# KTC-Security-Circle/3d-matching

Measured on AMD Instinct MI355X. Metric: ICP iterations/sec + RANSAC hypotheses/sec, 100k↔100k pts, 1/2/4/8 GPU, higher is better.
Workload: dtype fp16-split MFMA NN screen + fp32 scan, exact fp64 NN decision, fp64 terms/solve; 1 GPU; cfg1: 100000<->100000 synthetic pair per GPU, 50 point-to-plane ICP iterations, brute-force NN (r=0.12), 1 GPU; ns=100000, nt_per_gpu=100000, parallelism=single, comm=none, comm_ranks=1

## Files before the change

### 3d-matching_amd/csrc/api.cpp

```cpp
#include <cfloat>
#include <chrono>
#include <hip/hip_runtime.h>
#include <string.h>

#include <algorithm>
#include <cmath>
#include <string>
#include <memory>
#include <mutex>
#include <unordered_map>
#include <vector>

#include "linalg.h"
#include "m3d_internal.h"
#include "ddmath.h"

using namespace m3d;

int m3d_fail(m3d_ctx* ctx, int code, const std::string& msg) {
  if (ctx) ctx->err = msg;
  return code;
}

KTimer::KTimer(m3d_ctx* c, int kid, hipStream_t s) : ctx(c), id(kid), st(s) {
// ... 1261 lines not shown
      if (e != hipSuccess) grc = m3d_fail(ctx, M3D_ERR_HIP, std::string("grid fp64 points: ") + hipGetErrorString(e));
    }
    if (!grc && params->nn_method == M3D_NN_BRUTE && tg->mf16 == nullptr) {
      hipError_t e = build_mfma_tiles(tgt, const_cast<Grid*>(tg), &ctx->tmp, nullptr);
      if (e != hipSuccess) grc = m3d_fail(ctx, M3D_ERR_HIP, std::string("mfma tiles: ") + hipGetErrorString(e));
    }
    if (!grc) {
      cand_cap = heavy_cap(params, coarse_max_occ);
      const size_t n1 = (size_t)std::max<int64_t>(src->n, 1);
      Carve cv;
      cv.add(&s->state, 1);
      if (params->nn_method == M3D_NN_BRUTE) nn_plan_shape(src->n, &s->nn_qblocks, &s->nn_budget);
      if (s->nn_qblocks > 0) {
        cv.add(&s->nn_cnt, (size_t)s->nn_qblocks);
        cv.add(&s->nn_seen, (size_t)s->nn_qblocks);
        cv.add(&s->nn_table, (size_t)s->nn_budget);
      }
      cv.add(&s->keys, n1);
      cv.add(&s->near2, n1);
      cv.add(&s->dprev, n1);
      cv.add(&s->ld64, n1);
      cv.add(&s->lidx, n1);
      cv.add(&s->corr, n1);
      cv.add(&s->partials, (size_t)(terms_blocks(src->n) * kTermSlots + kTermSlots));
      if (cand_cap > 0) {
        cv.add(&s->hlist, n1);
        cv.add(&s->hcnt, kDeferWords);
        s->hcap = (int32_t)n1;
      }
      cv.add(&s->pcd64, 3 * n1);
      size_t tot = 0;
      hipError_t e = run_arena ? ctx->run.reserve(cv.bytes()) : cv.alloc(&s->block, &tot, nullptr);
      if (e != hipSuccess) grc = m3d_fail(ctx, M3D_ERR_OOM, "device allocation failed (ICP loop arrays)");
      if (!grc && run_arena) cv.place(ctx->run.base);
    }
    if (!grc && s->hcnt != nullptr &&
        hipMemsetAsync(s->hcnt, 0, kDeferWords * sizeof(uint32_t), nullptr) != hipSuccess)
      grc = m3d_fail(ctx, M3D_ERR_HIP, "loop arrays: deferral counter");
    if (!grc && s->nn_cnt != nullptr &&
        hipMemsetAsync(s->nn_cnt, 0, (size_t)s->nn_qblocks * sizeof(uint32_t), nullptr) != hipSuccess)
      grc = m3d_fail(ctx, M3D_ERR_HIP, "loop arrays: NN plan counters");
    if (!grc) {
      hipError_t e = hipStreamSynchronize(nullptr);
      if (e != hipSuccess) grc = m3d_fail(ctx, M3D_ERR_HIP, std::string("loop setup: ") + hipGetErrorString(e));
    }
    if (grc) {
// ... 1217 lines not shown
  const int32_t forced = 2;
  HIPX(s->ctx, hipMemcpyAsync(s->nn_table, table.data(), sizeof(uint32_t) * table.size(), hipMemcpyHostToDevice, S(stream)));
  HIPX(s->ctx, hipMemcpyAsync(&s->state->plan_ok, &forced, sizeof(forced), hipMemcpyHostToDevice, S(stream)));
  HIPX(s->ctx, hipStreamSynchronize(S(stream)));
  return M3D_OK;
}

int m3d_debug_icp_nn_plan_read(m3d_icp* s, uint32_t* counts, uint32_t* table, int32_t* shape3, void* stream) {
  if (!s || !shape3) return M3D_ERR_INVALID;
  shape3[0] = s->nn_qblocks;
  shape3[1] = s->nn_budget;
  shape3[2] = 0;
  if (s->nn_qblocks <= 0) return M3D_OK;
  Touch tch{s->ctx, S(stream)};
  if (counts)
    HIPX(s->ctx, hipMemcpyAsync(counts, s->nn_seen, sizeof(uint32_t) * (size_t)s->nn_qblocks, hipMemcpyDeviceToHost, S(stream)));
  if (table)
    HIPX(s->ctx, hipMemcpyAsync(table, s->nn_table, sizeof(uint32_t) * (size_t)s->nn_budget, hipMemcpyDeviceToHost, S(stream)));
  HIPX(s->ctx, hipMemcpyAsync(&shape3[2], &s->state->plan_ok, sizeof(int32_t), hipMemcpyDeviceToHost, S(stream)));
  HIPX(s->ctx, hipStreamSynchronize(S(stream)));
  return M3D_OK;
}

}
```

### 3d-matching_amd/csrc/icp.hip

```cpp
#include <float.h>

#include <algorithm>
#include <string>
#include <type_traits>
#include <vector>
#include <stdlib.h>

#include "lds_dma.h"
#include "linalg.h"
#include "m3d_internal.h"
#include "nnkey.h"

namespace m3d {

constexpr int kTermsBlock = 512;
constexpr double kU = 5.9604644775390625e-08;
constexpr double kU64 = 1.1102230246251565e-16;


struct FrameParams {
  double cs[3], ct[3];
  double pinf, qinf;
  double s16;
  int shared;
// ... 199 lines not shown
      for (int y = 0; y < 3; ++y) acc[6 + 3 * x + y] += pc[x] * qc[y];
    }
  }
}

struct TermsArgs {
  double* pcd64;
  const float4* src32;
  int64_t ns;
  const double* tgt64;
  const double* nrm64;
  const double* rec64;
  int64_t nt_shard, off;
  const int64_t* keys;
  uint32_t* near2;
  GridDev g;
  const int32_t* claim;
  const int64_t* dmin;
  int64_t* dprev;
  int32_t* corr;
  int est;
  double c[3];
  int64_t* reset_keys;
};

#if M3D_TAIL_CLOCK
__device__ unsigned long long g_tail_clock[3 * 4096 + 24];
#endif
#if M3D_TERMS_CLOCK
__device__ unsigned long long g_terms_clock[4096 * 8];
#define M3D_TPH(k)                               \
  do {                                           \
    __builtin_amdgcn_s_waitcnt(0);               \
    tph_[k] = __builtin_amdgcn_s_memrealtime();  \
  } while (0)
#else
#define M3D_TPH(k) \
  do {             \
  } while (0)
#endif
template <bool kWT, int kEst>
__device__ __forceinline__ void terms_block(const TermsArgs& a, const IcpState* __restrict__ s,
                                            double* __restrict__ partials) {
  __shared__ double red[kTermSlots][kTermsBlock / kWave];
#if M3D_TERMS_CLOCK
  unsigned long long tph_[8];
// ... 58 lines not shown
#endif
      qx[u] = qy[u] = qz[u] = 0.0f;
      if (amb[u]) xform32(s->Rt32, a.src32[ii[u]], qx[u], qy[u], qz[u]);
      bj[u] = -1;
      bd[u] = 0.0;
    }
    resolve_wave(amb[0], a.g, a.tgt64, a.off, qx[0], qy[0], qz[0], X[0], vs[0], s->r2, bj[0], bd[0]);
#pragma unroll
    for (int u = 0; u < kP; ++u) {
      if (amb[u]) {
        gj[u] = bj[u];
        d2[u] = bd[u];
      } else if (valid[u] && key_real(k1[u])) {
        const int64_t c = (int64_t)(uint32_t)k1[u];
        if (c >= a.off && c < a.off + a.nt_shard) {
          gj[u] = c;
          fixed[u] = false;
        }
      }
    }
  }
  M3D_TPH(2);
  double tq[kP][3], tn[kP][3];
#pragma unroll
  for (int u = 0; u < kP; ++u) {
    const bool own = valid[u] && gj[u] >= a.off && gj[u] < a.off + a.nt_shard;
    const int64_t l = own ? gj[u] - a.off : 0;
    if (a.nt_shard == 0) {
      for (int k = 0; k < 3; ++k) tq[u][k] = tn[u][k] = 0.0;
    } else if (a.rec64 != nullptr) {
      const double4 r0 = reinterpret_cast<const double4*>(a.rec64)[2 * l];
      const double4 r1 = reinterpret_cast<const double4*>(a.rec64)[2 * l + 1];
      tq[u][0] = r0.x;
      tq[u][1] = r0.y;
      tq[u][2] = r0.z;
      tn[u][0] = r0.w;
      tn[u][1] = r1.x;
      tn[u][2] = r1.y;
    } else {
#pragma unroll
      for (int k = 0; k < 3; ++k) {
        tq[u][k] = a.tgt64[3 * l + k];
        tn[u][k] = kEst == M3D_EST_POINT_TO_PLANE ? a.nrm64[3 * l + k] : 0.0;
      }
    }
  }
  M3D_TPH(3);
#pragma unroll
  for (int u = 0; u < kP; ++u) {
    if (!valid[u]) continue;
    if (!fixed[u]) {
      const double d = d2_64(vs[u], tq[u]);
      if (d < s->r2) {
        d2[u] = d;
      } else {
        gj[u] = -1;
      }
    }
    const int64_t i = ii[u];
    if (a.corr != nullptr) a.corr[i] = (int32_t)gj[u];
    if (gj[u] < a.off || gj[u] >= a.off + a.nt_shard) continue;
    terms_add<kEst>(acc, vs[u], tq[u], tn[u], d2[u], a.c);
  }
  M3D_TPH(4);
  const int lane = threadIdx.x & (kWave - 1), wave = threadIdx.x / kWave;
  {
    double v[32];
#pragma unroll
    for (int k = 0; k < 32; ++k) v[k] = k < 30 ? acc[k] : 0.0;
    const double w = wave_transpose_sum32(v, lane);
    if ((lane & 1) == 0) red[lane >> 1][wave] = w;
  }
  M3D_TPH(5);
  __syncthreads();
  M3D_TPH(6);
  if (threadIdx.x < kTermSlots) {
    double v = 0.0;
    if (threadIdx.x < 30)
      for (int w = 0; w < kTermsBlock / kWave; ++w) v += red[threadIdx.x][w];
    double* dst = partials + (int64_t)blockIdx.x * kTermSlots + threadIdx.x;
    if (kWT)
      __hip_atomic_store(reinterpret_cast<unsigned long long*>(dst), __double_as_longlong(v),
                         __ATOMIC_RELAXED, __HIP_MEMORY_SCOPE_AGENT);
// ... 665 lines not shown
  copy_points_kernel<<<(unsigned)((n + 255) / 256), 256, 0, st>>>(s->state, s->pcd64, s->src->slot, n, dst);
  return hipGetLastError();
}

hipError_t launch_val_states(const m3d_icp* s, const double* T_dev, const int32_t* list, int64_t n,
                             IcpState* states, hipStream_t st) {
  if (n == 0) return hipSuccess;
  val_states_kernel<<<(unsigned)((n + 63) / 64), 64, 0, st>>>(states, T_dev, list, n,
                                                              s->max_dist * s->max_dist, frame_of(s));
  return hipGetLastError();
}

hipError_t launch_icp_keyinit(const m3d_icp* s, int64_t off, hipStream_t st, int64_t q0, int64_t q1) {
  const int64_t ns = q1 < 0 ? s->src->n : q1;
  if (ns <= q0) return hipSuccess;
  keyinit_kernel<<<(unsigned)((ns - q0 + 255) / 256), 256, 0, st>>>(
      s->src->xyz32, ns, s->tgt->xyz32, s->tgt->n, off, s->state, s->corr, s->dprev, s->keys,
      s->near2, q0);
  return hipGetLastError();
}


__global__ __launch_bounds__(256) void pack_rec_kernel(const double* __restrict__ xyz,
                                                       const double* __restrict__ nrm, int64_t n,
                                                       double* __restrict__ rec) {
  const int64_t i = (int64_t)blockIdx.x * 256 + threadIdx.x;
  if (i >= n) return;
  double r[8];
  for (int k = 0; k < 3; ++k) {
    r[k] = xyz[3 * i + k];
    r[3 + k] = nrm != nullptr ? nrm[3 * i + k] : 0.0;
  }
  r[6] = r[7] = 0.0;
  for (int k = 0; k < 8; ++k) rec[8 * i + k] = r[k];
}

hipError_t ensure_target_rec(const m3d_cloud* c, hipStream_t st) {
  if (c->rec64 != nullptr || c->n == 0) return hipSuccess;
  double* rec = nullptr;
  hipError_t e = block_alloc(reinterpret_cast<void**>(&rec), sizeof(double) * 8 * c->n, st);
  if (e != hipSuccess) return e;
  pack_rec_kernel<<<(unsigned)((c->n + 255) / 256), 256, 0, st>>>(c->xyz64, c->nrm64, c->n, rec);
  e = hipGetLastError();
  if (e != hipSuccess) {
    block_release(rec);
    return e;
  }
  c->rec64 = rec;
  return hipSuccess;
}

__global__ __launch_bounds__(256) void pack_pts64_kernel(const float4* __restrict__ pts,
                                                         const double* __restrict__ xyz, int64_t n,
                                                         double4* __restrict__ out) {
  const int64_t k = (int64_t)blockIdx.x * 256 + threadIdx.x;
  if (k >= n) return;
  const int32_t j = __float_as_int(pts[k].w);
  out[k] = make_double4(xyz[3 * (int64_t)j], xyz[3 * (int64_t)j + 1], xyz[3 * (int64_t)j + 2],
                        __longlong_as_double((long long)j));
}

hipError_t build_grid_pts64(const m3d_cloud* c, Grid* g, hipStream_t st) {
  if (g->pts64 != nullptr || g->n_pts == 0) return hipSuccess;
  double4* p = nullptr;
  hipError_t e = block_alloc(reinterpret_cast<void**>(&p), sizeof(double4) * g->n_pts, st);
// ... 10 lines not shown
}

static TermsArgs terms_args(const m3d_icp* s, int64_t off, const int32_t* claim,
                            const int64_t* dmin, bool reset_keys) {
  TermsArgs a;
  a.pcd64 = s->pcd64;
  a.src32 = s->src->xyz32;
  a.ns = s->src->n;
  a.tgt64 = s->tgt->xyz64;
  a.nrm64 = s->tgt->nrm64;
  a.rec64 = s->tgt->rec64;
  a.nt_shard = s->tgt->n;
  a.off = off;
  a.keys = s->keys;
  a.near2 = s->near2;
  a.g = s->tgrid->dev;
  a.claim = claim;
  a.dmin = dmin;
  a.dprev = claim != nullptr ? s->dprev : nullptr;
  a.corr = s->corr;
  a.est = s->params.estimation;
  for (int k = 0; k < 3; ++k) a.c[k] = s->src->center[k];
  a.reset_keys = reset_keys ? s->keys : nullptr;
  return a;
}

hipError_t launch_icp_terms_mode(const m3d_icp* s, int64_t off, const int32_t* claim,
                                 const int64_t* dmin, hipStream_t st) {
  const int64_t ns = s->src->n;
  if (ns == 0) return hipMemsetAsync(s->partials, 0, sizeof(double) * kTermSlots, st);
  const TermsArgs ta = terms_args(s, off, claim, dmin, false);
  const unsigned nb = (unsigned)s->nblocks;
  with_est(ta.est, [&](auto e) {
    terms_kernel<decltype(e)::value><<<nb, kTermsBlock, 0, st>>>(ta, s->state, s->partials);
  });
  return hipGetLastError();
}

static void launch_reduce_groups(const m3d_icp* s, double* sums, int do_solve, hipStream_t st) {
  const SolveParams sp = do_solve ? solve_params(s) : SolveParams{};
  with_est(do_solve ? s->params.estimation : M3D_EST_POINT_TO_PLANE, [&](auto e) {
    reduce_groups_kernel<decltype(e)::value><<<kReduceGroups, kTermSlots, 0, st>>>(
        s->partials, s->nblocks, sums, s->state, sp, do_solve);
  });
}

// ... 135 lines not shown
```

### 3d-matching_amd/csrc/m3d_internal.h

```cpp
#pragma once

#include <hip/hip_runtime.h>
#include <stdint.h>

#include <algorithm>
#include <string>
#include <utility>
#include <functional>
#include <memory>
#include <mutex>
#include <vector>

#include "../../include/m3d.h"
#include "nn_plan.h"

#define M3D_CONST __attribute__((address_space(4)))

namespace m3d {

constexpr int kWave = 64;

struct alignas(64) HypF32 {
  float r[9];
  float t[3];
// ... 243 lines not shown
  const m3d_cloud* user_src = nullptr;
  const m3d_cloud* tgt = nullptr;
  m3d_icp_params params{};
  double max_dist = 0.0;
  void* block = nullptr;
  m3d::IcpState* state = nullptr;
  int64_t* keys = nullptr;
  uint32_t* near2 = nullptr;
  int64_t* dprev = nullptr;
  int64_t* ld64 = nullptr;
  int32_t* lidx = nullptr;
  int32_t* hlist = nullptr;
  uint32_t* hcnt = nullptr;
  int32_t hcap = 0;
  int32_t cand_cap = 0;
  int32_t scan_xchunk = 0;
  bool keys_clean = false;
  uint32_t* nn_cnt = nullptr;
  uint32_t* nn_seen = nullptr;
  uint32_t* nn_table = nullptr;
  int32_t nn_qblocks = 0;
  int32_t nn_budget = 0;
  int32_t* corr = nullptr;
  double* pcd64 = nullptr;
  double* partials = nullptr;
  double* sums = nullptr;
  int64_t nblocks = 0;
  const m3d::Grid* sgrid = nullptr;
  const m3d::Grid* tgrid = nullptr;
  int64_t ns_total = 0;
  bool xready_tgt = false;
  bool xready_src = false;
  int64_t* xdk = nullptr;
  int32_t* xcl = nullptr;
  double* xsums = nullptr;
  hipStream_t cap_stream = nullptr;
  hipGraphExec_t graph[2] = {nullptr, nullptr};
  int32_t graph_n[2] = {-1, -1};
  bool graph_kc_out[2] = {false, false};
  int32_t seen_n[2] = {-1, -1};
  bool graph_off = false;
};

int m3d_fail(m3d_ctx* ctx, int code, const std::string& msg);

struct KTimer {
// ... 197 lines not shown
```

### 3d-matching_amd/csrc/nn_brute.hip

```cpp
#include <algorithm>

#include "lds_dma.h"
#include "m3d_internal.h"
#include "nnkey.h"

#ifndef M3D_NN_BRUTE_PLAN_TU
#define M3D_NN_BRUTE_PLAN_TU 0
#endif
#ifndef M3D_NN_CLOCK
#define M3D_NN_CLOCK 0
#endif
#define M3D_NN_TU_MAIN (!M3D_NN_BRUTE_PLAN_TU)
#define M3D_NN_TU_PLAN_KERNEL (M3D_NN_BRUTE_PLAN_TU ? !M3D_NN_CLOCK : M3D_NN_CLOCK)
#if M3D_NN_TU_MAIN || M3D_NN_TU_PLAN_KERNEL

namespace m3d {

typedef _Float16 half8 __attribute__((ext_vector_type(8)));
typedef float floatx16 __attribute__((ext_vector_type(16)));

constexpr int kMG = 2;
constexpr int kMTile = 256;
constexpr int kTH = 4;
constexpr int kMTilePad = 1024;
// ... 112 lines not shown
    block_release(g->mf32);
    block_release(g->mfbox);
    g->mf16 = nullptr;
    g->mf32 = nullptr;
    g->mfbox = nullptr;
    return e;
  }
  g->mf_npad = n_pad;
  pack16_sorted_kernel<<<(unsigned)((n_pad + 255) / 256), 256, 0, st>>>(
      g->pts, perm, c->xyz32, n, n_pad, (float)c->s16, g->mf16, g->mf32);
  tile_box_kernel<<<(unsigned)(n_pad / kMTile), kMTile, 0, st>>>(g->mf32, g->mfbox);
  return hipGetLastError();
}

#endif

struct SeedArgs {
  const int32_t* prev;
  const float4* tgt;
  int64_t nt;
  int on;
};

__device__ __forceinline__ int64_t start_key(const SeedArgs& sa, const IcpState* __restrict__ s,
                                             int64_t i, float4 p, float qx, float qy, float qz,
                                             int64_t off, const int64_t* __restrict__ keys) {
  return sa.on ? seed_key(s, i, p, qx, qy, qz, sa.tgt, sa.nt, off, sa.prev, nullptr) : keys[i];
}

struct NnSlice {
  unsigned x, y, S;
};
struct NnPlan {
  const uint32_t* table;
  uint32_t* cnt;
  int nq, S;
};

__device__ __forceinline__ bool publish_k1(const SeedArgs& sa, unsigned y, uint64_t k1, bool changed) {
  return changed || (sa.on && y == 0 && key_real(k1));
}

__device__ void nn_slice_scan(const float4* __restrict__ src32, int64_t ns, const float4* __restrict__ tgt32,
                              int64_t jb, int64_t je, int64_t off, const IcpState* __restrict__ s,
                              int64_t* __restrict__ keys, uint32_t* __restrict__ near2,
                              const SeedArgs& sa, int64_t q0, unsigned bsx, unsigned bsy) {
  const float* Rt = s->Rt32;
  const float r2_hi = s->r2_hi;
  for (int qs = threadIdx.x; qs < kMQueries; qs += kMBlock) {
    const int64_t slot = q0 + (int64_t)bsx * kMQueries + qs;
    if (slot >= ns) return;
    const int64_t i = slot;
    float qx, qy, qz;
    const float4 p = src32[i];
    xform32(Rt, p, qx, qy, qz);
    const int64_t key = start_key(sa, s, i, p, qx, qy, qz, off, keys);
    uint64_t k1 = key == kKeyNone ? make_key(r2_hi, 0xFFFFFFFFu) : (uint64_t)key;
    float k1d = key_real_d2(k1), n2 = kInf;
    const uint64_t k10 = k1;
    for (int64_t j = jb; j < je; ++j) {
      const float4 t = tgt32[j];
      if (__float_as_int(t.w) < 0) continue;
      const float d2 = d2f(qx, qy, qz, t.x, t.y, t.z);
      if (d2 <= r2_hi) near_push(k1, k1d, n2, make_key(d2, (uint32_t)(off + __float_as_int(t.w))), d2);
    }
    const bool pk = publish_k1(sa, bsy, k1, k1 != k10);
    if (pk || n2 < kInf) near_publish((unsigned long long*)&keys[i], &near2[i], k1, n2, pk);
  }
}

__device__ __forceinline__ void nn_push_rows(const float4 (&t)[16], int64_t off, float qx, float qy, float qz,
                                             float r2_hi, uint64_t& k1, float& k1d, float& n2) {
#pragma unroll
  for (int reg = 0; reg < 16; ++reg) {
    const float d2 = d2f(qx, qy, qz, t[reg].x, t[reg].y, t[reg].z);
    const uint64_t kc = make_key(d2, (uint32_t)(off + __float_as_int(t[reg].w)));
    if (d2 <= r2_hi) near_push(k1, k1d, n2, kc, d2);
  }
}
// ... 21 lines not shown
  x |= __builtin_amdgcn_mov_dpp(x, 0x128, 0xF, 0xF, false);
  return (uint32_t)(__builtin_amdgcn_readlane(x, 0) | __builtin_amdgcn_readlane(x, 16) |
                    __builtin_amdgcn_readlane(x, 32) | __builtin_amdgcn_readlane(x, 48));
}

template <bool kMax>
__device__ __forceinline__ float wave_minmax(float v) {
  const auto mm = [](float a, float b) { return kMax ? fmaxf(a, b) : fminf(a, b); };
  v = mm(v, __int_as_float(__builtin_amdgcn_mov_dpp(__float_as_int(v), 0xB1, 0xF, 0xF, false)));
  v = mm(v, __int_as_float(__builtin_amdgcn_mov_dpp(__float_as_int(v), 0x4E, 0xF, 0xF, false)));
  v = mm(v, __int_as_float(xor4_dpp(__float_as_int(v))));
  v = mm(v, __int_as_float(__builtin_amdgcn_mov_dpp(__float_as_int(v), 0x128, 0xF, 0xF, false)));
  const int x = __float_as_int(v);
  return mm(mm(__int_as_float(__builtin_amdgcn_readlane(x, 0)), __int_as_float(__builtin_amdgcn_readlane(x, 16))),
            mm(__int_as_float(__builtin_amdgcn_readlane(x, 32)), __int_as_float(__builtin_amdgcn_readlane(x, 48))));
}

#ifndef M3D_NN_CULL
#define M3D_NN_CULL 1
#endif
#ifndef M3D_NN_REACH
#define M3D_NN_REACH 1
#endif
#ifndef M3D_NN_DEFER_BATCH
#define M3D_NN_DEFER_BATCH 1
#endif
#ifndef M3D_NN_DEFER_FILTER
#define M3D_NN_DEFER_FILTER 1
#endif
#if M3D_NN_CLOCK
constexpr int kClkBlocks = 16384, kClkWords = 8;
__device__ unsigned long long g_nn_clock[kClkWords * kClkBlocks];
#endif
struct QBox {
  float lo[3], hi[3], X;
};
__device__ __forceinline__ bool box_out_of_reach(const QBox& q, const float4& tlo, const float4& thi) {
  const float gx = fmaxf(0.0f, fmaxf(q.lo[0] - thi.x, tlo.x - q.hi[0]));
  const float gy = fmaxf(0.0f, fmaxf(q.lo[1] - thi.y, tlo.y - q.hi[1]));
  const float gz = fmaxf(0.0f, fmaxf(q.lo[2] - thi.z, tlo.z - q.hi[2]));
  return d2f(gx, gy, gz, 0.0f, 0.0f, 0.0f) > q.X;
}
__device__ __forceinline__ bool point_out_of_reach(float qx, float qy, float qz, float X, const float (&lo)[3],
                                                   const float (&hi)[3]) {
  const float gx = fmaxf(0.0f, fmaxf(qx - hi[0], lo[0] - qx));
  const float gy = fmaxf(0.0f, fmaxf(qy - hi[1], lo[1] - qy));
// ... 6 lines not shown
constexpr uint64_t kGMask = (kSub == 64) ? ~0ull : ((1ull << kSub) - 1ull);
constexpr int kDefer = 16;
static_assert(kMBlock == 2 * kMTile, "one 16-B operand half per thread per half tile");
static_assert(kSub * kMG <= 64, "hit mask holds every (group, sub-tile)");
static_assert(kSub == 32, "one 32-bit hit record per group and tile");
static_assert(kMBlock / 64 == 8, "eight wave boxes, lanes ^1 ^2 ^4");

struct QState {
  float qx, qy, qz, qq;
  int64_t qi;
  uint64_t k1;
  float k1d, n2;
  half8 bq;
};

__device__ __forceinline__ uint64_t group_mask(uint32_t bits) {
  uint64_t m = 0;
#pragma unroll
  for (int g = 0; g < kMG; ++g)
    if ((bits >> g) & 1u) m |= kGMask << (g * kSub);
  return m;
}

__device__ __forceinline__ float load_query(QState& q, QBox& lq, int64_t slot, int h,
                                            const float4* __restrict__ src32, int64_t ns,
                                            const IcpState* __restrict__ s, const SeedArgs& sa, int64_t off,
                                            const int64_t* __restrict__ keys) {
  const float* Rt = s->Rt32;
  const float r2_hi = s->r2_hi, S = s->mfma_scale;
  const int64_t i = slot < ns ? slot : -1;
  q.qi = i;
  q.n2 = kInf;
  float X = -1.0f;
  if (i >= 0) {
    const float4 p = src32[i];
    xform32(Rt, p, q.qx, q.qy, q.qz);
    const int64_t key = start_key(sa, s, i, p, q.qx, q.qy, q.qz, off, keys);
    q.k1 = key == kKeyNone ? make_key(r2_hi, 0xFFFFFFFFu) : (uint64_t)key;
    X = search_bound(key_d2(q.k1), s->band_e, r2_hi);
    lq.lo[0] = fminf(lq.lo[0], q.qx);
    lq.lo[1] = fminf(lq.lo[1], q.qy);
    lq.lo[2] = fminf(lq.lo[2], q.qz);
    lq.hi[0] = fmaxf(lq.hi[0], q.qx);
    lq.hi[1] = fmaxf(lq.hi[1], q.qy);
    lq.hi[2] = fmaxf(lq.hi[2], q.qz);
    lq.X = fmaxf(lq.X, X);
  } else {
    q.qx = q.qy = q.qz = 0.0f;
    q.k1 = (uint64_t)kKeyNone;
  }
  q.k1d = key_real_d2(q.k1);
  q.qq = fmaf(q.qz, q.qz, fmaf(q.qy, q.qy, q.qx * q.qx));
  _Float16 ah, al, bh, bl, ch, cl;
  split16(-2.0f * S * q.qx, ah, al);
  split16(-2.0f * S * q.qy, bh, bl);
  split16(-2.0f * S * q.qz, ch, cl);
  const _Float16 one = (_Float16)1.0f, zero = (_Float16)0.0f;
  q.bq = h == 0 ? half8{ah, al, ah, bh, bl, bh, ch, cl} : half8{ch, one, one, zero, zero, zero, zero, zero};
  return X;
}
// ... 195 lines not shown
  uint32_t m = 0;
#pragma unroll
  for (int reg = 15; reg >= 0; --reg) m = __builtin_amdgcn_alignbit(m, __float_as_uint(v[reg]), 31);
  return m;
}
__device__ __forceinline__ void nn_push_hits(uint32_t m, const float4* rows, int64_t off, int h, float qx,
                                             float qy, float qz, float r2_hi, uint64_t& k1, float& k1d,
                                             float& n2) {
  while (m != 0) {
    const int reg = __builtin_ctz(m);
    m &= m - 1;
    const float4 t = rows[(reg & 3) + 8 * (reg >> 2) + 4 * h];
    push_within(k1, k1d, n2, d2f(qx, qy, qz, t.x, t.y, t.z), r2_hi, (uint32_t)(off + __float_as_int(t.w)));
  }
}

template <bool kPlan>
__device__ __forceinline__ void nn_mfma_body(const float4* __restrict__ src32, int64_t ns,
                                             const uint4* __restrict__ tgt16, const float4* __restrict__ tgt32,
                                             const float4* __restrict__ tbox, int64_t nt_pad, int64_t off,
                                             const IcpState* __restrict__ s, int64_t* __restrict__ keys,
                                             uint32_t* __restrict__ near2, const SeedArgs& sa, int64_t q0,
                                             const NnPlan& pl) {
  if (s->done) return;
#if M3D_NN_CLOCK
  const unsigned long long clk0 = __builtin_amdgcn_s_memrealtime();
#endif
  NnSlice bs{0u, 0u, 0u};
  if (kPlan && pl.table != nullptr) {
    if (s->plan_ok) {
      const uint32_t e = pl.table[blockIdx.x];
      if (e == kPlanEmpty) return;
      bs = NnSlice{plan_x(e), plan_y(e), plan_S(e)};
    } else {
      const unsigned y = blockIdx.x / (unsigned)pl.nq;
      if (y >= (unsigned)pl.S) return;
      bs = NnSlice{blockIdx.x - y * (unsigned)pl.nq, y, (unsigned)pl.S};
    }
  }
  if (!s->mfma_ok) {
    const int64_t tstep = (int64_t)(kPlan ? bs.S : gridDim.y) * kTT;
    for (int64_t t0 = (int64_t)(kPlan ? bs.y : blockIdx.y) * kTT; t0 < nt_pad; t0 += tstep)
      nn_slice_scan(src32, ns, tgt32, t0, min(nt_pad, t0 + kTT), off, s, keys, near2, sa, q0,
                    kPlan ? bs.x : blockIdx.x, kPlan ? bs.y : blockIdx.y);
    return;
  }
  __shared__ uint4 t16[2][2][kTT];
  __shared__ uint64_t dlist[kMBlock / 64][kDefer];
  __shared__ uint32_t dtile[kMBlock / 64][kDefer];
  __shared__ float4 qbox[kMBlock / 64][2];
  __shared__ uint64_t rslot[2][kMBlock / 64];
#if M3D_NN_CLOCK
  __shared__ uint32_t clk_slow, clk_ticket;
  __shared__ unsigned long long clk_exit;
  if (threadIdx.x == 0) {
    clk_slow = 0;
    clk_ticket = 0;
    clk_exit = 0;
  }
  uint32_t clk_halves = 0;
#endif
  uint32_t kept = 0;
  __shared__ uint32_t slice_xy;
  if (kPlan && threadIdx.x == 0) slice_xy = bs.x | (bs.y << 16);
  const int lane = threadIdx.x & 63, wave = threadIdx.x >> 6;
  const int c = lane & 31, h = lane >> 5;
  const float r2_hi = s->r2_hi, eps = s->screen_eps_m, S = s->mfma_scale, be = s->band_e;
  const float S2 = S * S;

  QState q[kMG];
  uint32_t act = 0;
  uint32_t force = 0;
  uint32_t chg = 0;
  QBox lq{{kInf, kInf, kInf}, {-kInf, -kInf, -kInf}, -1.0f};
#pragma unroll
  for (int g = 0; g < kMG; ++g) {
    const int64_t slot = q0 + (kPlan ? (int64_t)bs.x : (int64_t)blockIdx.x) * kMQueries + (wave * kMG + g) * 32 + c;
    const float X = load_query(q[g], lq, slot, h, src32, ns, s, sa, off, keys);
    if (q[g].qi >= 0) act |= 1u << g;
    if (__any(refresh_threshold(q[g], h, X, eps, S2))) force |= 1u << g;
  }
  const floatx16 zacc = {0.0f, 0.0f, 0.0f, 0.0f, 0.0f, 0.0f, 0.0f, 0.0f,
                         0.0f, 0.0f, 0.0f, 0.0f, 0.0f, 0.0f, 0.0f, 0.0f};
  uint32_t dfr = 0;
#pragma unroll
  for (int g = 0; g < kMG; ++g)
    if (!((force >> g) & 1u) && __all(q[g].qi < 0 || key_real(q[g].k1))) dfr |= 1u << g;
  int dn = 0;
  uint64_t dmask = group_mask(dfr);
  dmask = ((uint64_t)(uint32_t)__builtin_amdgcn_readfirstlane((int)(dmask >> 32)) << 32) |
          (uint32_t)__builtin_amdgcn_readfirstlane((int)(uint32_t)dmask);

  const QBox bx = reduce_boxes(lq, qbox, lane, wave);
  const int ntile = (int)(nt_pad / kTT);
  const ReachArgs ra{q, act, be, r2_hi, rslot, wave};
  TileCursor cur{tbox, qbox[wave], bx, lane, ntile, (int)(kPlan ? bs.S : gridDim.y), (int)(kPlan ? bs.y : blockIdx.y), 0, 0};
  cur.cull_round(ra);
  int t0, t1;
  uint32_t h0, h1;
  cur.next(t0, h0, ra);
  if (t0 < ntile) stage_tile(t16[0], tgt16, nt_pad, t0, false);
// ... 256 lines not shown
  return hipMemcpyFromSymbol(out, HIP_SYMBOL(m3d::g_nn_clock), sizeof(unsigned long long) * (size_t)n) == hipSuccess ? 0 : -1;
}
namespace m3d {
#endif
static bool icp_nn_uses_mfma(const m3d_icp* s) {
  return s->tgrid != nullptr && s->tgrid->mf16 != nullptr;
}

bool icp_nn_range_ok(const m3d_icp* s) {
  if (s->params.nn_method == M3D_NN_GRID) return s->sgrid != nullptr && s->sgrid->mpts != nullptr;
  return icp_nn_uses_mfma(s);
}

hipError_t launch_icp_nn(const m3d_icp* s, int64_t off, bool self_seed, hipStream_t st, int64_t q0,
                         int64_t q1) {
  const int64_t ns = q1 < 0 ? s->src->n : q1;
  if (ns <= q0 || s->tgt->n == 0) return hipSuccess;
  const Grid* tg = s->tgrid;
  const int64_t tt = (int64_t)kTH * kMTile;
  if (!icp_nn_uses_mfma(s) || tg->mf_npad % tt != 0) return hipErrorInvalidValue;
  const int64_t slots = nn_resident_slots();
  const int64_t bx = (ns - q0 + kMQueries - 1) / kMQueries;
  const int64_t gy = nn_grid_y(bx, tg->mf_npad / tt, slots, M3D_NN_CULL != 0);
  const SeedArgs sa{s->corr, s->tgt->xyz32, s->tgt->n, self_seed ? 1 : 0};
  const bool planned = nn_plan_on() && s->nn_qblocks > 0 && q0 == 0 && ns == s->src->n && bx == s->nn_qblocks &&
                       bx * gy <= s->nn_budget;
  if (planned)
    return launch_nn_plan_kernel((unsigned)s->nn_budget, st, s->src->xyz32, ns, tg->mf16, tg->mf32, tg->mfbox,
                                 tg->mf_npad, off, s->state, s->keys, s->near2, sa, q0,
                                 NnPlan{s->nn_table, s->nn_cnt, (int)bx, (int)gy});
  nn_mfma_kernel<<<dim3((unsigned)bx, (unsigned)gy), kMBlock, 0, st>>>(
        s->src->xyz32, ns, tg->mf16, tg->mf32, tg->mfbox, tg->mf_npad, off, s->state, s->keys, s->near2, sa, q0);
  return hipGetLastError();
}

int64_t nn_resident_slots() {
  static const int64_t slots = [] {
    int dev = 0, per = 0;
    hipDeviceProp_t p;
    if (hipGetDevice(&dev) != hipSuccess || hipGetDeviceProperties(&p, dev) != hipSuccess) return (int64_t)0;
    if (hipOccupancyMaxActiveBlocksPerMultiprocessor(&per, nn_mfma_kernel, kMBlock, 0) != hipSuccess)
      return (int64_t)0;
    const int pp = nn_plan_kernel_blocks_per_cu();
    per = per > 0 ? per : 1;
    if (pp > 0 && pp < per) per = pp;
    return (int64_t)p.multiProcessorCount * per;
  }();
// ... 35 lines not shown
```

### 3d-matching_amd/csrc/nnkey.h

```cpp
#pragma once

#include <hip/hip_runtime.h>
#include <stdint.h>

#include "m3d_internal.h"

namespace m3d {

__device__ __forceinline__ float d2f(float qx, float qy, float qz, float tx, float ty, float tz) {
  const float dx = qx - tx, dy = qy - ty, dz = qz - tz;
  return fmaf(dz, dz, fmaf(dy, dy, dx * dx));
}

__device__ __forceinline__ void xform32(const float* Rt, float4 p, float& x, float& y, float& z) {
  x = fmaf(Rt[0], p.x, fmaf(Rt[1], p.y, fmaf(Rt[2], p.z, Rt[9])));
  y = fmaf(Rt[3], p.x, fmaf(Rt[4], p.y, fmaf(Rt[5], p.z, Rt[10])));
  z = fmaf(Rt[6], p.x, fmaf(Rt[7], p.y, fmaf(Rt[8], p.z, Rt[11])));
}

__device__ __forceinline__ void q64_of(const double* __restrict__ T, const double* __restrict__ p,
                                       double q[3]) {
  q[0] = ((T[0] * p[0] + T[1] * p[1]) + T[2] * p[2]) + T[3];
  q[1] = ((T[4] * p[0] + T[5] * p[1]) + T[6] * p[2]) + T[7];
  q[2] = ((T[8] * p[0] + T[9] * p[1]) + T[10] * p[2]) + T[11];
// ... 352 lines not shown
                                              const float4* __restrict__ tgt32, int64_t nt_shard,
                                              int64_t off, const int64_t* __restrict__ dprev) {
  if (j < 0) return kKeyNone;
  if (j >= off && j < off + nt_shard) {
    const float4 t = tgt32[j - off];
    const float d2 = d2f(qx, qy, qz, t.x, t.y, t.z);
    return d2 <= s->r2_hi ? (int64_t)make_key(d2, (uint32_t)j) : kKeyNone;
  }
  if (!s->bound_ok || dprev == nullptr) return kKeyNone;
  const int64_t dp = dprev[i];
  if (dp == kKeyNone) return kKeyNone;
  return bound_key(s, __double2float_ru(__longlong_as_double(dp)), p, qx, qy, qz);
}

__device__ __forceinline__ int64_t seed_key(const IcpState* __restrict__ s, int64_t i, float4 p,
                                            float qx, float qy, float qz,
                                            const float4* __restrict__ tgt32, int64_t nt_shard,
                                            int64_t off, const int32_t* __restrict__ prev,
                                            const int64_t* __restrict__ dprev) {
  if (prev == nullptr) return kKeyNone;
  return seed_key_j(s, (int64_t)prev[i], i, p, qx, qy, qz, tgt32, nt_shard, off, dprev);
}

}
```

### 3d-matching_amd/m3d/_lib.py

```python

from __future__ import annotations

import ctypes as C
import os
from pathlib import Path

LIB_PATH = Path(__file__).resolve().parent / "libm3d.so"

M3D_OK = 0
M3D_ERR_INVALID = -1
M3D_ERR_HIP = -2
M3D_ERR_OOM = -3
M3D_ERR_NODEVICE = -4
M3D_ERR_COMM = -5

HYP_OK, HYP_DEGENERATE, HYP_NONFINITE = 0, 1, 2
SCORE_SQUARED, SCORE_NORM = 0, 1
EST_POINT_TO_POINT, EST_POINT_TO_PLANE = 0, 1
KERNEL_NN, KERNEL_SCORE, KERNEL_KABSCH, KERNEL_TERMS, KERNEL_LOOP, KERNEL_COMM = 0, 1, 2, 3, 4, 5
ICP_NO_SPLIT = 2
NN_BRUTE, NN_GRID = 0, 1
EVAL_INFORMATION = 1
COMM_ID_BYTES = 128
DT_I32, DT_I64, DT_F64 = 0, 1, 2
# ... 150 lines not shown
    "m3d_model_resolution": (C.c_int, [vp, vp, C.POINTER(dbl), vp]),
    "m3d_compute_iss_keypoints": (C.c_int, [vp, vp, C.POINTER(IssParams), C.POINTER(IssResult), vp, vp, vp, vp]),
    "m3d_feature_correspondences": (C.c_int, [vp, vp, i64, vp, i64, i32, i32, dbl, vp,
                                              C.POINTER(i64), vp]),
    "m3d_ransac_on_correspondences": (C.c_int, [vp, vp, vp, vp, i64, C.POINTER(FeatureRansacParams),
                                                C.POINTER(FeatureRansacResult), vp, vp]),
    "m3d_comm_unique_id": (C.c_int, [C.POINTER(C.c_uint8)]),
    "m3d_comm_init": (C.c_int, [vp, C.POINTER(C.c_uint8), C.c_int, C.c_int, C.POINTER(vp)]),
    "m3d_comm_destroy": (None, [vp]),
    "m3d_comm_allreduce": (C.c_int, [vp, vp, i64, C.c_int, C.c_int, vp]),
    "m3d_icp_shard_steps": (C.c_int, [vp, vp, i64, i32, vp]),
    "m3d_icp_source_shard_steps": (C.c_int, [vp, vp, i32, vp]),
    "m3d_ransac_best_allreduce": (C.c_int, [vp, vp, i64, vp, vp]),
    "m3d_ransac_run_sharded": (C.c_int, [vp, vp, vp, C.POINTER(RansacParams), C.POINTER(RansacResult), vp]),
    "m3d_comm_poisoned": (C.c_int, [vp]),
    "m3d_debug_comm_inject": (C.c_int, [vp, C.c_int]),
    "m3d_debug_acos_cr": (C.c_int, [vp, C.c_int64, vp]),
    "m3d_debug_acos_device": (C.c_int, [vp, vp, C.c_int64, vp, C.c_int, vp]),
    "m3d_debug_block_cache_fill": (C.c_int, [C.c_int]),
    "m3d_debug_icp_defer_count": (C.c_int, [vp, C.c_uint32, vp]),
    "m3d_debug_nn_plan_host": (C.c_int, [vp, C.c_int64, C.c_int64, C.c_int64, C.c_int64, vp]),
    "m3d_debug_icp_nn_plan": (C.c_int, [vp, vp, C.c_int64, vp]),
    "m3d_debug_icp_nn_plan_read": (C.c_int, [vp, vp, vp, vp, vp]),
    "m3d_parse_ascii_rows": (C.c_int, [C.c_char_p, C.c_size_t, i64, i32, C.POINTER(dbl),
                                       C.POINTER(C.c_size_t)]),
    "m3d_format_ascii_rows": (C.c_int, [C.POINTER(dbl), i64, i32, vp, C.c_size_t, C.POINTER(C.c_size_t)]),
    "m3d_merge_vertices": (C.c_int, [C.POINTER(dbl), i64, C.POINTER(dbl), C.POINTER(i32), C.POINTER(i64)]),
    "m3d_content_keys": (C.c_int, [C.POINTER(vp), C.POINTER(C.c_size_t), i32, C.POINTER(u64)]),
    "m3d_debug_xxh64": (u64, [vp, C.c_size_t, u64]),
    "m3d_debug_xxh3_128": (C.c_int, [vp, C.c_size_t, C.POINTER(u64)]),
    "m3d_debug_kabsch3_host":(C.c_int, [C.POINTER(dbl), C.POINTER(dbl), C.POINTER(dbl)]),
    "m3d_debug_ldlt6_host": (C.c_int, [C.POINTER(dbl), C.POINTER(dbl), C.POINTER(dbl)]),
    "m3d_debug_sym3_eigenvalues_host": (C.c_int, [C.POINTER(dbl), C.POINTER(dbl)]),
}

_lib = None


class M3DError(RuntimeError):
    pass


class M3DCommError(M3DError):
    """A peer rank failed, or the communicator was aborted after a failure (M3D_ERR_COMM)."""


# ... 40 lines not shown
```

### include/m3d.h

```cpp
#ifndef M3D_H_
#define M3D_H_

#include <stddef.h>
#include <stdint.h>

#ifdef __cplusplus
extern "C" {
#endif

#define M3D_ABI_VERSION 13

#define M3D_OK 0
#define M3D_ERR_INVALID (-1)
#define M3D_ERR_HIP (-2)
#define M3D_ERR_OOM (-3)
#define M3D_ERR_NODEVICE (-4)
#define M3D_ERR_COMM (-5)

#define M3D_HYP_OK 0
#define M3D_HYP_DEGENERATE 1
#define M3D_HYP_NONFINITE 2

#define M3D_SCORE_SQUARED 0
#define M3D_SCORE_NORM 1
// ... 292 lines not shown
  double corres_ratio;
} m3d_feature_ransac_result;

int m3d_ransac_on_correspondences(m3d_ctx* ctx, const m3d_cloud* src, const m3d_cloud* tgt,
                                  const int32_t* corr, int64_t nc,
                                  const m3d_feature_ransac_params* params,
                                  m3d_feature_ransac_result* out, int32_t* corr_set_out,
                                  void* stream);

int m3d_debug_kabsch3_host(const double* src9, const double* tgt9, double* T16);
int m3d_debug_ldlt6_host(const double* A36, const double* b6, double* x6);
int m3d_debug_sym3_eigenvalues_host(const double* sym6, double* lam3);
uint64_t m3d_debug_xxh64(const void* p, size_t len, uint64_t seed);
int m3d_debug_xxh3_128(const void* p, size_t len, uint64_t* out2);
int m3d_debug_comm_inject(m3d_comm* c, int what);
int m3d_debug_acos_cr(const double* u, int64_t n, double* out);
int m3d_debug_acos_device(m3d_ctx* ctx, const double* u, int64_t n, double* out, int mode, void* stream);
int m3d_debug_block_cache_fill(int byte);
int m3d_debug_icp_defer_count(m3d_icp* s, uint32_t count, void* stream);
int m3d_debug_nn_plan_host(const uint32_t* counts, int64_t n, int64_t budget, int64_t smax, int64_t ntiles,
                           uint32_t* out);
int m3d_debug_icp_nn_plan(m3d_icp* s, const int32_t* S, int64_t n, void* stream);
int m3d_debug_icp_nn_plan_read(m3d_icp* s, uint32_t* counts, uint32_t* table, int32_t* shape3, void* stream);


int m3d_parse_ascii_rows(const char* buf, size_t len, int64_t rows, int32_t cols, double* out,
                         size_t* consumed);
int m3d_format_ascii_rows(const double* data, int64_t rows, int32_t cols, char* out, size_t cap,
                          size_t* written);
int m3d_merge_vertices(const double* xyz, int64_t n, double* uniq, int32_t* inverse,
                       int64_t* n_unique);
int m3d_content_keys(const void* const* bufs, const size_t* lens, int32_t n, uint64_t* keys);

#ifdef __cplusplus
}
#endif
#endif
```

Baseline: 19720 ICP iter/s (100k src x 100k tgt per GPU).

## Store per-source seed records in terms pass to avoid gathered target loads in NN

The terms kernel now writes a per-source float4 seed record holding the matched target's fp32 xyz and index. The fp32 xyz comes from padding slots in the packed target record, so the terms kernel gets it without an extra load. The brute NN kernel then reads this record contiguously instead of a dependent gather through corr into the target array. The NN kernel also hoists its IcpState flag reads and plan table entry into scalar registers at entry, and batches its query loads. This adds one float4 store per source per iteration and extra memory in exchange for removing the random gather on the next NN pass.

```diff
diff --git a/3d-matching_amd/csrc/api.cpp b/3d-matching_amd/csrc/api.cpp
--- a/3d-matching_amd/csrc/api.cpp
+++ b/3d-matching_amd/csrc/api.cpp
@@ -1307,6 +1307,7 @@
       cv.add(&s->ld64, n1);
       cv.add(&s->lidx, n1);
       cv.add(&s->corr, n1);
+      if (params->nn_method == M3D_NN_BRUTE) cv.add(&s->seed, n1);
       cv.add(&s->partials, (size_t)(terms_blocks(src->n) * kTermSlots + kTermSlots));
       if (cand_cap > 0) {
         cv.add(&s->hlist, n1);
@@ -2570,4 +2571,22 @@
   return M3D_OK;
 }
 
-}
+int m3d_debug_icp_seed_read(m3d_icp* s, float* seed, int32_t* corr, float* tgt32, int32_t* info2, void* stream) {
+  if (!s || !info2) return M3D_ERR_INVALID;
+  CHECK_ARG(s->ctx, s->seed != nullptr && s->tgt->rec64 != nullptr,
+            "this loop keeps no seed records (brute-force NN on a non-empty target only)");
+  info2[0] = s->keys_clean ? 1 : 0;
+  Touch tch{s->ctx, S(stream)};
+  HIPX(s->ctx, hipMemcpyAsync(&info2[1], &s->state->mfma_ok, sizeof(int32_t), hipMemcpyDeviceToHost, S(stream)));
+  const size_t ns = (size_t)s->src->n, nt = (size_t)s->tgt->n;
+  if (seed && ns > 0)
+    HIPX(s->ctx, hipMemcpyAsync(seed, s->seed, sizeof(float4) * ns, hipMemcpyDeviceToHost, S(stream)));
+  if (corr && ns > 0)
+    HIPX(s->ctx, hipMemcpyAsync(corr, s->corr, sizeof(int32_t) * ns, hipMemcpyDeviceToHost, S(stream)));
+  if (tgt32)
+    HIPX(s->ctx, hipMemcpyAsync(tgt32, s->tgt->xyz32, sizeof(float4) * nt, hipMemcpyDeviceToHost, S(stream)));
+  HIPX(s->ctx, hipStreamSynchronize(S(stream)));
+  return M3D_OK;
+}
+
+}
diff --git a/3d-matching_amd/csrc/icp.hip b/3d-matching_amd/csrc/icp.hip
--- a/3d-matching_amd/csrc/icp.hip
+++ b/3d-matching_amd/csrc/icp.hip
@@ -245,6 +245,7 @@
   int est;
   double c[3];
   int64_t* reset_keys;
+  float4* seed;
 };
 
 #if M3D_TAIL_CLOCK
@@ -349,8 +350,10 @@
   }
   M3D_TPH(2);
   double tq[kP][3], tn[kP][3];
+  double pad[kP][2];
 #pragma unroll
   for (int u = 0; u < kP; ++u) {
+    pad[u][0] = pad[u][1] = 0.0;
     const bool own = valid[u] && gj[u] >= a.off && gj[u] < a.off + a.nt_shard;
     const int64_t l = own ? gj[u] - a.off : 0;
     if (a.nt_shard == 0) {
@@ -364,6 +367,8 @@
       tn[u][0] = r0.w;
       tn[u][1] = r1.x;
       tn[u][2] = r1.y;
+      pad[u][0] = r1.z;
+      pad[u][1] = r1.w;
     } else {
 #pragma unroll
       for (int k = 0; k < 3; ++k) {
@@ -386,6 +391,10 @@
     }
     const int64_t i = ii[u];
     if (a.corr != nullptr) a.corr[i] = (int32_t)gj[u];
+    if (kWT && a.seed != nullptr) {
+      a.seed[i] = make_float4(__int_as_float(__double2loint(pad[u][0])), __int_as_float(__double2hiint(pad[u][0])),
+                              __int_as_float(__double2loint(pad[u][1])), __int_as_float((int32_t)gj[u]));
+    }
     if (gj[u] < a.off || gj[u] >= a.off + a.nt_shard) continue;
     terms_add<kEst>(acc, vs[u], tq[u], tn[u], d2[u], a.c);
   }
@@ -1097,7 +1106,8 @@
 
 
 __global__ __launch_bounds__(256) void pack_rec_kernel(const double* __restrict__ xyz,
-                                                       const double* __restrict__ nrm, int64_t n,
+                                                       const double* __restrict__ nrm,
+                                                       const float4* __restrict__ xyz32, int64_t n,
                                                        double* __restrict__ rec) {
   const int64_t i = (int64_t)blockIdx.x * 256 + threadIdx.x;
   if (i >= n) return;
@@ -1106,7 +1116,9 @@
     r[k] = xyz[3 * i + k];
     r[3 + k] = nrm != nullptr ? nrm[3 * i + k] : 0.0;
   }
-  r[6] = r[7] = 0.0;
+  const float4 p = xyz32[i];
+  r[6] = __hiloint2double(__float_as_int(p.y), __float_as_int(p.x));
+  r[7] = __hiloint2double(__float_as_int(p.w), __float_as_int(p.z));
   for (int k = 0; k < 8; ++k) rec[8 * i + k] = r[k];
 }
 
@@ -1115,7 +1127,7 @@
   double* rec = nullptr;
   hipError_t e = block_alloc(reinterpret_cast<void**>(&rec), sizeof(double) * 8 * c->n, st);
   if (e != hipSuccess) return e;
-  pack_rec_kernel<<<(unsigned)((c->n + 255) / 256), 256, 0, st>>>(c->xyz64, c->nrm64, c->n, rec);
+  pack_rec_kernel<<<(unsigned)((c->n + 255) / 256), 256, 0, st>>>(c->xyz64, c->nrm64, c->xyz32, c->n, rec);
   e = hipGetLastError();
   if (e != hipSuccess) {
     block_release(rec);
@@ -1172,6 +1184,7 @@
   a.est = s->params.estimation;
   for (int k = 0; k < 3; ++k) a.c[k] = s->src->center[k];
   a.reset_keys = reset_keys ? s->keys : nullptr;
+  a.seed = reset_keys && claim == nullptr && off == 0 && a.rec64 != nullptr ? s->seed : nullptr;
   return a;
 }
 
diff --git a/3d-matching_amd/csrc/m3d_internal.h b/3d-matching_amd/csrc/m3d_internal.h
--- a/3d-matching_amd/csrc/m3d_internal.h
+++ b/3d-matching_amd/csrc/m3d_internal.h
@@ -289,6 +289,7 @@
   int32_t nn_qblocks = 0;
   int32_t nn_budget = 0;
   int32_t* corr = nullptr;
+  float4* seed = nullptr;
   double* pcd64 = nullptr;
   double* partials = nullptr;
   double* sums = nullptr;
diff --git a/3d-matching_amd/csrc/nn_brute.hip b/3d-matching_amd/csrc/nn_brute.hip
--- a/3d-matching_amd/csrc/nn_brute.hip
+++ b/3d-matching_amd/csrc/nn_brute.hip
@@ -158,10 +158,14 @@
   int on;
 };
 
-__device__ __forceinline__ int64_t start_key(const SeedArgs& sa, const IcpState* __restrict__ s,
-                                             int64_t i, float4 p, float qx, float qy, float qz,
-                                             int64_t off, const int64_t* __restrict__ keys) {
-  return sa.on ? seed_key(s, i, p, qx, qy, qz, sa.tgt, sa.nt, off, sa.prev, nullptr) : keys[i];
+__device__ __forceinline__ float4 seed_rec_prev(const SeedArgs& sa, int64_t i, int64_t off) {
+  const int64_t j = sa.prev[i];
+  float4 r = make_float4(0.0f, 0.0f, 0.0f, __int_as_float(-1));
+  if (j >= off && j < off + sa.nt) {
+    r = sa.tgt[j - off];
+    r.w = __int_as_float((int32_t)j);
+  }
+  return r;
 }
 
 struct NnSlice {
@@ -190,7 +194,8 @@
     float qx, qy, qz;
     const float4 p = src32[i];
     xform32(Rt, p, qx, qy, qz);
-    const int64_t key = start_key(sa, s, i, p, qx, qy, qz, off, keys);
+    const int64_t key = sa.on == 0 ? keys[i]
+                                   : seed_key_rec(s, sa.on == 2 ? sa.tgt[i] : seed_rec_prev(sa, i, off), qx, qy, qz);
     uint64_t k1 = key == kKeyNone ? make_key(r2_hi, 0xFFFFFFFFu) : (uint64_t)key;
     float k1d = key_real_d2(k1), n2 = kInf;
     const uint64_t k10 = k1;
@@ -258,6 +263,12 @@
 #ifndef M3D_NN_REACH
 #define M3D_NN_REACH 1
 #endif
+#ifndef M3D_NN_ENTRY
+#define M3D_NN_ENTRY 1
+#endif
+#ifndef M3D_NN_SEED_REC
+#define M3D_NN_SEED_REC 1
+#endif
 #ifndef M3D_NN_DEFER_BATCH
 #define M3D_NN_DEFER_BATCH 1
 #endif
@@ -310,9 +321,8 @@
   return m;
 }
 
-__device__ __forceinline__ float load_query(QState& q, QBox& lq, int64_t slot, int h,
-                                            const float4* __restrict__ src32, int64_t ns,
-                                            const IcpState* __restrict__ s, const SeedArgs& sa, int64_t off,
+__device__ __forceinline__ float load_query(QState& q, QBox& lq, int64_t slot, int h, float4 p, float4 rec,
+                                            int64_t ns, const IcpState* __restrict__ s, const SeedArgs& sa,
                                             const int64_t* __restrict__ keys) {
   const float* Rt = s->Rt32;
   const float r2_hi = s->r2_hi, S = s->mfma_scale;
@@ -321,9 +331,8 @@
   q.n2 = kInf;
   float X = -1.0f;
   if (i >= 0) {
-    const float4 p = src32[i];
     xform32(Rt, p, q.qx, q.qy, q.qz);
-    const int64_t key = start_key(sa, s, i, p, q.qx, q.qy, q.qz, off, keys);
+    const int64_t key = sa.on ? seed_key_rec(s, rec, q.qx, q.qy, q.qz) : keys[i];
     q.k1 = key == kKeyNone ? make_key(r2_hi, 0xFFFFFFFFu) : (uint64_t)key;
     X = search_bound(key_d2(q.k1), s->band_e, r2_hi);
     lq.lo[0] = fminf(lq.lo[0], q.qx);
@@ -565,14 +574,27 @@
                                              const IcpState* __restrict__ s, int64_t* __restrict__ keys,
                                              uint32_t* __restrict__ near2, const SeedArgs& sa, int64_t q0,
                                              const NnPlan& pl) {
+#if M3D_NN_ENTRY
+  uint32_t e_tab = kPlanEmpty;
+  if (kPlan && pl.table != nullptr) e_tab = pl.table[blockIdx.x];
+  int32_t st_done = s->done, st_plan = s->plan_ok, st_mfma = s->mfma_ok;
+  asm volatile("" : "+s"(st_done), "+s"(st_plan), "+s"(st_mfma), "+s"(e_tab));
+  if (st_done) return;
+#else
   if (s->done) return;
+#endif
 #if M3D_NN_CLOCK
   const unsigned long long clk0 = __builtin_amdgcn_s_memrealtime();
 #endif
   NnSlice bs{0u, 0u, 0u};
   if (kPlan && pl.table != nullptr) {
+#if M3D_NN_ENTRY
+    if (st_plan) {
+      const uint32_t e = e_tab;
+#else
     if (s->plan_ok) {
       const uint32_t e = pl.table[blockIdx.x];
+#endif
       if (e == kPlanEmpty) return;
       bs = NnSlice{plan_x(e), plan_y(e), plan_S(e)};
     } else {
@@ -581,7 +603,11 @@
       bs = NnSlice{blockIdx.x - y * (unsigned)pl.nq, y, (unsigned)pl.S};
     }
   }
+#if M3D_NN_ENTRY
+  if (!st_mfma) {
+#else
   if (!s->mfma_ok) {
+#endif
     const int64_t tstep = (int64_t)(kPlan ? bs.S : gridDim.y) * kTT;
     for (int64_t t0 = (int64_t)(kPlan ? bs.y : blockIdx.y) * kTT; t0 < nt_pad; t0 += tstep)
       nn_slice_scan(src32, ns, tgt32, t0, min(nt_pad, t0 + kTT), off, s, keys, near2, sa, q0,
@@ -616,10 +642,31 @@
   uint32_t force = 0;
   uint32_t chg = 0;
   QBox lq{{kInf, kInf, kInf}, {-kInf, -kInf, -kInf}, -1.0f};
+  const int64_t slot0 = q0 + (kPlan ? (int64_t)bs.x : (int64_t)blockIdx.x) * kMQueries + wave * kMG * 32 + c;
+  float4 qp[kMG], qr[kMG];
 #pragma unroll
   for (int g = 0; g < kMG; ++g) {
-    const int64_t slot = q0 + (kPlan ? (int64_t)bs.x : (int64_t)blockIdx.x) * kMQueries + (wave * kMG + g) * 32 + c;
-    const float X = load_query(q[g], lq, slot, h, src32, ns, s, sa, off, keys);
+    const int64_t slot = slot0 + g * 32;
+    qp[g] = src32[slot < ns ? slot : 0];
+    qr[g] = make_float4(0.0f, 0.0f, 0.0f, 0.0f);
+  }
+  if (sa.on == 2) {
+#pragma unroll
+    for (int g = 0; g < kMG; ++g) {
+      const int64_t slot = slot0 + g * 32;
+      qr[g] = sa.tgt[slot < ns ? slot : 0];
+    }
+  } else if (sa.on) {
+#pragma unroll
+    for (int g = 0; g < kMG; ++g) {
+      const int64_t slot = slot0 + g * 32;
+      qr[g] = seed_rec_prev(sa, slot < ns ? slot : 0, off);
+    }
+  }
+#pragma unroll
+  for (int g = 0; g < kMG; ++g) {
+    const int64_t slot = slot0 + g * 32;
+    const float X = load_query(q[g], lq, slot, h, qp[g], qr[g], ns, s, sa, keys);
     if (q[g].qi >= 0) act |= 1u << g;
     if (__any(refresh_threshold(q[g], h, X, eps, S2))) force |= 1u << g;
   }
@@ -922,7 +969,8 @@
   const int64_t slots = nn_resident_slots();
   const int64_t bx = (ns - q0 + kMQueries - 1) / kMQueries;
   const int64_t gy = nn_grid_y(bx, tg->mf_npad / tt, slots, M3D_NN_CULL != 0);
-  const SeedArgs sa{s->corr, s->tgt->xyz32, s->tgt->n, self_seed ? 1 : 0};
+  const bool by_rec = M3D_NN_SEED_REC != 0 && self_seed && off == 0 && s->tgt->rec64 != nullptr && s->seed != nullptr;
+  const SeedArgs sa{s->corr, by_rec ? s->seed : s->tgt->xyz32, s->tgt->n, by_rec ? 2 : self_seed ? 1 : 0};
   const bool planned = nn_plan_on() && s->nn_qblocks > 0 && q0 == 0 && ns == s->src->n && bx == s->nn_qblocks &&
                        bx * gy <= s->nn_budget;
   if (planned)
diff --git a/3d-matching_amd/csrc/nnkey.h b/3d-matching_amd/csrc/nnkey.h
--- a/3d-matching_amd/csrc/nnkey.h
+++ b/3d-matching_amd/csrc/nnkey.h
@@ -398,4 +398,12 @@
   return seed_key_j(s, (int64_t)prev[i], i, p, qx, qy, qz, tgt32, nt_shard, off, dprev);
 }
 
-}
+__device__ __forceinline__ int64_t seed_key_rec(const IcpState* __restrict__ s, float4 rec, float qx, float qy,
+                                                float qz) {
+  const int32_t j = __float_as_int(rec.w);
+  if (j < 0) return kKeyNone;
+  const float d2 = d2f(qx, qy, qz, rec.x, rec.y, rec.z);
+  return d2 <= s->r2_hi ? (int64_t)make_key(d2, (uint32_t)j) : kKeyNone;
+}
+
+}
diff --git a/3d-matching_amd/m3d/_lib.py b/3d-matching_amd/m3d/_lib.py
--- a/3d-matching_amd/m3d/_lib.py
+++ b/3d-matching_amd/m3d/_lib.py
@@ -196,6 +196,7 @@
     "m3d_debug_nn_plan_host": (C.c_int, [vp, C.c_int64, C.c_int64, C.c_int64, C.c_int64, vp]),
     "m3d_debug_icp_nn_plan": (C.c_int, [vp, vp, C.c_int64, vp]),
     "m3d_debug_icp_nn_plan_read": (C.c_int, [vp, vp, vp, vp, vp]),
+    "m3d_debug_icp_seed_read": (C.c_int, [vp, vp, vp, vp, vp, vp]),
     "m3d_parse_ascii_rows": (C.c_int, [C.c_char_p, C.c_size_t, i64, i32, C.POINTER(dbl),
                                        C.POINTER(C.c_size_t)]),
     "m3d_format_ascii_rows": (C.c_int, [C.POINTER(dbl), i64, i32, vp, C.c_size_t, C.POINTER(C.c_size_t)]),
diff --git a/include/m3d.h b/include/m3d.h
--- a/include/m3d.h
+++ b/include/m3d.h
@@ -338,6 +338,7 @@
                            uint32_t* out);
 int m3d_debug_icp_nn_plan(m3d_icp* s, const int32_t* S, int64_t n, void* stream);
 int m3d_debug_icp_nn_plan_read(m3d_icp* s, uint32_t* counts, uint32_t* table, int32_t* shape3, void* stream);
+int m3d_debug_icp_seed_read(m3d_icp* s, float* seed, int32_t* corr, float* tgt32, int32_t* info2, void* stream);
 
 
 int m3d_parse_ascii_rows(const char* buf, size_t len, int64_t rows, int32_t cols, double* out,
```

New measurement: 20480 ICP iter/s (100k src x 100k tgt per GPU) (median of 6 runs). +3.9%, better.
